# hhguo/MSMC-TTS

Hardware: AMD Instinct MI355X
Metric: mel-frames/sec MSMC-VQ-GAN train step (GAN phase) (higher is better)
Workload: dtype bf16

## Files before the change

### include/msmc_hip_debug.h

```cpp
#ifndef MSMC_HIP_DEBUG_H
#define MSMC_HIP_DEBUG_H
#include "msmc_hip.h"
#ifdef __cplusplus
extern "C" {
#endif

void msmc_vq_set_shortlist_ablate(int mask);

void msmc_vq_set_variant(int v);

void msmc_vq_wide_set_split(int wc);

void msmc_triple_wide_set_frames(int ft);

void msmc_conv_set_gather4_grid(int n);
void msmc_conv_set_gather4_grouping(int on);
void msmc_conv_set_pipeline(int on);
void msmc_conv_set_wgrad_split(int n);
void msmc_conv_set_wgrad_tpw(int n);
void msmc_conv_set_wgrad_generation(int n);
void msmc_conv_set_gather_generation(int n);
void msmc_conv_set_narrow(int on);

void msmc_conv_set_grouping(int on);

void msmc_conv_set_wgrad4_ablate(int mask);

const char* msmc_vq_last_kernel(void);
const char* msmc_loss_last_kernel(void);
void msmc_prof_enable(int on);
int msmc_prof_count(void);
int msmc_prof_read(int i, char* name, int cap, float* ms);
const char* msmc_conv_last_kernel(void);
long msmc_conv_launch_count(void);
#ifdef __cplusplus
}
#endif
#endif
```

### msmc-tts_amd/csrc/conv.hip

```cpp
#include <msmc_rt.hpp>
#include <msmc_hip.h>
#include <msmc_hip_debug.h>
#include "conv_common.inc"

extern "C" void msmc_conv_set_pipeline(int on) { msmc_conv_pipeline_enabled = on; }
static int msmc_conv_narrow_when_small = 1;
extern "C" void msmc_conv_set_narrow(int on) { msmc_conv_narrow_when_small = on; }
extern "C" const char* msmc_conv_last_kernel(void) { return msmc_conv_last; }
extern "C" long msmc_conv_launch_count(void) { return msmc_conv_launches; }
extern "C" int msmc_conv_gather(const msmc_conv_desc* d, msmc_stream stream);
static int msmc_gather_generation = 2;
extern "C" void msmc_conv_set_gather_generation(int n) { msmc_gather_generation = n; }

template <int N>
MSMC_DEV void cv_ep(float (&v)[N], const unsigned int* mk, const unsigned int* r1, const unsigned int* r2, bool has_mask,
                    bool has_res, bool has_res2, float mslope, float odiv, float oslope) {
    if (has_mask) {
#pragma unroll
        for (int j = 0; j < N; ++j) {
            const float mj = __uint_as_float((j & 1) ? (mk[j >> 1] & 0xffff0000u) : (mk[j >> 1] << 16));
            v[j] = v[j] * (mj > 0.f ? 1.f : mslope);
        }
    }
    if (has_res) {
// ... 579 lines not shown
    const bool ovec = (d.Cout % VEC) == 0;
    const size_t img = (size_t)b * d.Hout * d.Wout;
    for (int e = tid; e < 128 * BNV; e += 256) {
        const int m = e / BNV, vcol = (e - m * BNV) * VEC;
        const int po = out_off[m], co = co0 + vcol;
        if (po < 0 || co >= d.Cout) continue;
        const size_t o = (img + po) * d.Cout + co;
        float v[VEC];
#pragma unroll
        for (int q = 0; q < VEC; ++q) v[q] = ot[m * OS + vcol + q] + ((d.bias && co + q < d.Cout) ? d.bias[co + q] : 0.f);
        alignas(16) T mk[VEC], r1[VEC], r2[VEC], ov[VEC];
        if (ovec) {
            if (mask) *(u32x4*)mk = *(const u32x4*)(mask + o);
            if (res) *(u32x4*)r1 = *(const u32x4*)(res + o);
            if (res2) *(u32x4*)r2 = *(const u32x4*)(res2 + o);
        } else {
#pragma unroll
            for (int q = 0; q < VEC; ++q) {
                const bool in = co + q < d.Cout;
                if (mask) mk[q] = in ? mask[o + q] : (T)0;
                if (res) r1[q] = in ? res[o + q] : (T)0;
                if (res2) r2[q] = in ? res2[o + q] : (T)0;
            }
        }
#pragma unroll
        for (int q = 0; q < VEC; ++q) {
            float x = v[q];
            if (mask) x = x * (Elt<T>::ld(&mk[q]) > 0.f ? 1.f : d.mask_slope);
            if (res) x = x + Elt<T>::ld(&r1[q]);
            if (res2) x = Elt<T>::ld(&r2[q]) + x;
            if (d.out_div != 1.f) x = x / d.out_div;
            if (d.out_slope != 1.f) x = x > 0.f ? x : x * d.out_slope;
            Elt<T>::st(&ov[q], x);
        }
        if (ovec) {
            *(u32x4*)(out + o) = *(const u32x4*)ov;
        } else {
#pragma unroll
            for (int q = 0; q < VEC; ++q)
                if (co + q < d.Cout) out[o + q] = ov[q];
        }
    }
}


template <typename T, int NT, int CKM, int SB>
__global__ __launch_bounds__(256, 2) void conv_gather2_kernel(msmc_conv_desc d, CvGeom G) {
    cv2_body<T, NT, CKM, SB>(d, G, blockIdx.x, blockIdx.y);
}

struct CvGroupArgs {
    int n;
    int first[MSMC_GROUP_MAX + 1];
    int nx[MSMC_GROUP_MAX];
    msmc_conv_desc d[MSMC_GROUP_MAX];
    CvGeom G[MSMC_GROUP_MAX];
};
template <typename T, int NT, int CKM, int SB>
__global__ __launch_bounds__(256, 2) void conv_gather2_group_kernel(CvGroupArgs a) {
    const int k = cv_group_member(a.first, a.n);
    const int id = blockIdx.x - a.first[k];
    cv2_body<T, NT, CKM, SB>(a.d[k], a.G[k], id % a.nx[k], id / a.nx[k]);
}

template <class F>
static int cv_family_dispatch(const msmc_conv_desc* descs, const typename F::Plan* pl, const int* members, int m,
                              msmc_stream stream) {
    typename F::Args a;
    int* first = F::head(a, m);
    int blocks = 0;
    size_t lds = 0;
    for (int k = 0; k < m; ++k) {
        const int j = members[k];
        first[k] = blocks;
        F::fill(a, k, descs[j], pl[j]);
        blocks += F::blocks(pl[j]);
        if (pl[j].lds > lds) lds = pl[j].lds;
    }
    first[m] = blocks;
    ++msmc_conv_launches;
    return F::dispatch(pl[members[0]], blocks, lds, stream, m == 1 ? &descs[members[0]] : nullptr, m == 1 ? nullptr : &a);
}
template <class F>
static int cv_family_group_launch(const msmc_conv_desc* descs, int n, msmc_stream stream, bool* done) {
    typename F::Plan pl[MSMC_GROUP_LIMIT];
    bool todo[MSMC_GROUP_LIMIT];
    int count = 0;
    for (int i = 0; i < n; ++i) {
        todo[i] = !done[i] && F::mine(&descs[i]);
        count += todo[i];
    }
    if (count < F::min_members) return 0;
    for (int i = 0; i < n; ++i) {
        if (!todo[i]) continue;
        int rc = F::plan(&descs[i], &pl[i], count < MSMC_GROUP_MAX ? count : MSMC_GROUP_MAX);
        if (rc) return rc;
        if (!pl[i].applies) return MSMC_E_SHAPE;
    }
    for (int i = 0; i < n; ++i) {
        if (!todo[i]) continue;
        int members[MSMC_GROUP_MAX], m = 0;
        for (int j = i; j < n && m < MSMC_GROUP_MAX; ++j) {
            if (!todo[j] || !F::same(pl[i], pl[j])) continue;
            members[m++] = j;
            todo[j] = false;
        }
        if (m == 1 && !F::lone_single) continue;
        for (int k = 0; k < m; ++k) done[members[k]] = true;
        int rc = cv_family_dispatch<F>(descs, pl, members, m, stream);
        if (rc) return rc;
    }
    return 0;
}

#include "gather3.inc"
#include "gather4.inc"
#include "gemm1.inc"
#include "gather5.inc"
#include "gather7.inc"
#include "gather6.inc"

template <typename T, int NT, int MT>
static int cv_try_pipe(const msmc_conv_desc* d, msmc_stream stream, bool* done) {
    constexpr int XS = Elt<T>::CK + Elt<T>::VEC, CKV = Elt<T>::CK / Elt<T>::VEC;
    CvGeom G;
    size_t lds;
    *done = false;
    int rc = cv_geometry(d, &G, sizeof(T), XS, 32 * NT, &lds, CV_BM * MT);
    if (rc) return rc;
    if (lds > 160 * 1024) return 0;
    if (G.IH * G.IW * CKV > 256 * CV_XLD || d->ntaps * 32 * NT * CKV > 256 * CV_WLD) return 0;
    dim3 grid((unsigned)(G.tilesX * G.tilesY * d->B), (unsigned)((d->Cout + 32 * NT - 1) / (32 * NT)));
    rc = msmc_allow_lds((const void*)conv_gather_pipe_kernel<T, NT, MT>, (int)lds);
    if (rc) return rc;
    MSMC_LAUNCH((conv_gather_pipe_kernel<T, NT, MT>), grid, dim3(256), lds, (msmc_stream_t)stream, *d, G);
    msmc_conv_last = msmc_prof_name(msmc_kname("conv_gather_pipe_kernel", EltName<T>::v, NT, MT));
    *done = true;
    return msmc_check_launch();
}

struct Cv2Plan {
    int applies;
    int nt, ckm, sb;
    CvGeom G;
    size_t lds;
    unsigned gx, gy;
};
template <typename T>
static int cv2_plan(const msmc_conv_desc* d, Cv2Plan* pl, int* narrow_nt) {
    constexpr int XS = Elt<T>::CK + Elt<T>::VEC;
    pl->applies = 0;
    int NT = d->Cout > 32 ? 2 : 1;
    if (NT == 2 && msmc_conv_narrow_when_small) {
        const long mt = ((long)d->QH * d->QW + CV_BM - 1) / CV_BM * d->B;
        const long wide = mt * ((d->Cout + 63) / 64);
        if (wide < MSMC_NUM_CU || (wide < 2 * MSMC_NUM_CU && d->Cin >= 256)) NT = 1;
    }
    *narrow_nt = NT;
    const int gen = d->variant > 0 ? d->variant : msmc_gather_generation;
    const bool sb8 = gen == 4 || gen == 5 || (d->variant == 0 && (long)d->ntaps * 32 * NT * (Elt<T>::CK / Elt<T>::VEC) > 1024);
    const bool ck1 = gen == 3 || gen == 5 || gen == 7;
    const bool want16 = gen == 6 || gen == 7;
    bool shallow = d->Cin < 4 * Elt<T>::CK || (d->Cin % Elt<T>::VEC) != 0 || gen >= 3 || d->variant == 2;
    if (want16 && (d->Cin % Elt<T>::VEC) != 0) return MSMC_E_SHAPE;
    if (!shallow && gen == 2) {
        const long points = (long)d->B * d->QH * d->QW;
        const long ntile = (d->Cout + 32 * NT - 1) / (32 * NT);
        shallow = (points / (CV_BM * 2)) * ntile < 2 * MSMC_NUM_CU;
    }
    if (!(gen >= 2 && shallow && (long)d->Hin * d->Win * d->Cin < (1L << 31) && (long)d->Hout * d->Wout < (1L << 31)))
        return 0;
    size_t unused;
    int rc = cv_geometry(d, &pl->G, sizeof(T), XS, 32, &unused);
    if (rc) return rc;
    const long npix = (long)pl->G.IH * pl->G.IW;
    const size_t tables = (((size_t)(npix + 128 + 16) * sizeof(int)) + 15) & ~(size_t)15;
    auto lds_of = [&](int nt, int ckm) {
        const size_t xs = (size_t)Elt<T>::CK * ckm + Elt<T>::VEC;
        const size_t stage = ((size_t)npix + (size_t)d->ntaps * 32 * nt) * xs * sizeof(T);
        const size_t epi = (size_t)128 * (32 * nt + 4) * sizeof(float);
        return tables + (stage > epi ? stage : epi);
    };
    int nt = NT;
    int ckm = (d->Cin >= 2 * Elt<T>::CK && (d->Cin % Elt<T>::VEC) == 0 && lds_of(nt, 2) <= 64 * 1024 && !ck1) ? 2 : 1;
    if (lds_of(nt, ckm) > 160 * 1024 && nt == 2) nt = 1;
    const size_t lds2 = lds_of(nt, ckm);
    const long chunk_vectors = (npix + (long)d->ntaps * 32 * nt) * (Elt<T>::CK * ckm / Elt<T>::VEC);
    const bool sb16 = want16 && chunk_vectors <= 16L * 256 && (d->Cin % Elt<T>::VEC) == 0;
    if (want16 && !sb16) return MSMC_E_SHAPE;
    if (lds2 > 160 * 1024) return 0;
    pl->applies = 1;
// ... 967 lines not shown
```

### msmc-tts_amd/csrc/gather6.inc

```
#define CV6_HEAD 768
#ifndef CV6_BATCH
#define CV6_BATCH 3
#endif
struct Cv6Run {
    int npoints, ntiles;
    int nsteps;
    int pitch;
    int nco;
    int cin, cinsh;
    unsigned int m_qpi, m_qw;
    int dymin, dymax, dxmin, dxmax;
};

MSMC_DEV int cv6_div(int n, int dv, unsigned int m) {
    if (dv == 1) return n;
    unsigned int q = __umulhi((unsigned int)n, m);
    if (q * (unsigned int)dv > (unsigned int)n) --q;
    return (int)q;
}

template <int NCO>
MSMC_DEV void cv6_body(const msmc_conv_desc& d, const Cv6Run& R, const int block, const int nblocks) {
    MSMC_DYN_LDS(smem);
    typedef unsigned short T;
    const int CIN = R.cin, cinsh = R.cinsh;
    const int g8sh = cinsh >= 3 ? cinsh - 3 : 0;
    int* tapdy = (int*)smem;
    int* tapdx = tapdy + 32;
    int* koff = tapdx + 32;
    char* wimg = smem + CV6_HEAD;
    const int tid = threadIdx.x, w = wave_uniform(tid >> 6), lane = tid & 63, li = lane & 31, g = lane >> 5;
    const int Cout = d.Cout, ntaps = d.ntaps, pitch = R.pitch;
    const int nk8 = (ntaps * CIN + 7) >> 3;

    for (int e = tid; e < 32 * NCO * (pitch >> 4); e += 256) *(u32x4*)(wimg + (size_t)e * 16) = u32x4{0u, 0u, 0u, 0u};
    if (tid < 32) {
        tapdy[tid] = tid < ntaps ? d.tap_dy[tid] : 0;
        tapdx[tid] = tid < ntaps ? d.tap_dx[tid] : 0;
    }
    if (tid < 128) {
        const int t = tid >> g8sh, cg = tid - (t << g8sh);
        koff[tid] = (CIN >= 8 && t < ntaps) ? (((d.tap_dy[t] * d.Win + d.tap_dx[t]) << cinsh) + cg * 8) : 0;
    }
    __syncthreads();
    if (CIN >= 8) {
        for (int e = tid; e < Cout * nk8; e += 256) {
            const int co = e / nk8, kk = e - co * nk8;
            const int t = kk >> g8sh, cg = kk - (t << g8sh);
            const u32x4 v = *(const u32x4*)((const T*)d.w + (((size_t)d.tap_w[t] * Cout + co) << cinsh) + cg * 8);
            *(u32x4*)(wimg + (size_t)co * pitch + kk * 16) = v;
        }
    } else {
        const int kreal = ntaps << cinsh;
        for (int e = tid; e < Cout * kreal; e += 256) {
            const int co = e / kreal, k = e - co * kreal;
            const int t = k >> cinsh, ci = k - (t << cinsh);
            *(T*)(wimg + (size_t)co * pitch + k * 2) = ((const T*)d.w)[(((size_t)d.tap_w[t] * Cout + co) << cinsh) + ci];
        }
    }
    __syncthreads();

    const T* xg = (const T*)d.x;
    const float slope = d.in_slope;
    const int qpi = d.QH * d.QW;
    const T* mask = (const T*)d.mask_src;
    const T* res = (const T*)d.res;
    const T* res2 = (const T*)d.res2;
    T* out = (T*)d.out;
    const float mslope = d.mask_slope, odiv = d.out_div, oslope = d.out_slope;
    const char* wrow = wimg + (size_t)li * pitch + g * 16;

    for (int tile = block * 4 + w; tile < R.ntiles; tile += nblocks * 4) {
        const int p = tile * 32 + li;
        const bool live = p < R.npoints;
        const int pc = live ? p : R.npoints - 1;
        const int b = cv6_div(pc, qpi, R.m_qpi), q = pc - b * qpi;
        const int qy = cv6_div(q, d.QW, R.m_qw), qx = q - qy * d.QW;
        const int iy0 = d.iy0 + qy * d.isy, ix0 = d.ix0 + qx * d.isx;
        const int xb = b * d.Hin;
        const bool inside_pt = live && iy0 + R.dymin >= 0 && iy0 + R.dymax < d.Hin && ix0 + R.dxmin >= 0 && ix0 + R.dxmax < d.Win;
        const bool fast = CIN >= 8 && !wave_any(!inside_pt);
        const T* xbase = xg + (long)((xb + iy0) * d.Win + ix0) * CIN;
        f32x16 acc[NCO];
#pragma unroll
        for (int c = 0; c < NCO; ++c)
#pragma unroll
            for (int r = 0; r < 16; ++r) acc[c][r] = 0.f;
        auto load_piece = [&](int ks) -> u32x4 {
            const int kk = 2 * ks + g;
            u32x4 v = {0u, 0u, 0u, 0u};
            if (kk >= nk8) return v;
            auto pixel = [&](int t, unsigned int& off) -> bool {
                int iy = iy0 + tapdy[t], ix = ix0 + tapdx[t];
                bool inside = live;
                if (d.pad_mode == 1) {
                    iy = reflect_index(iy, d.Hin);
                    ix = reflect_index(ix, d.Win);
                } else {
                    inside = inside && (iy >= 0) && (iy < d.Hin) && (ix >= 0) && (ix < d.Win);
                }
                off = (unsigned int)(((xb + iy) * d.Win + ix) << cinsh);
                return inside;
            };
            unsigned int off;
            if (CIN >= 8) {
                const int t = kk >> g8sh, cg = kk - (t << g8sh);
                if (pixel(t, off)) v = *(const u32x4*)(xg + (size_t)off + cg * 8);
            } else if (CIN == 4) {
#pragma unroll
                for (int tp = 0; tp < 2; ++tp) {
                    const int t = 2 * kk + tp;
                    if (t < ntaps && pixel(t, off)) {
                        const u32x2 h = *(const u32x2*)(xg + (size_t)off);
                        v[2 * tp] = h[0];
                        v[2 * tp + 1] = h[1];
                    }
                }
            } else {
#pragma unroll
                for (int tp = 0; tp < 4; ++tp) {
                    const int t = 4 * kk + tp;
                    if (t < ntaps && pixel(t, off)) v[tp] = *(const unsigned int*)(xg + (size_t)off);
                }
            }
            return v;
        };
        for (int s0 = 0; s0 < R.nsteps; s0 += CV6_BATCH) {
            u32x4 xf[CV6_BATCH];
            if (fast) {
#pragma unroll
                for (int u = 0; u < CV6_BATCH; ++u) {
                    const int kk = 2 * (s0 + u) + g;
                    xf[u] = u32x4{0u, 0u, 0u, 0u};
                    if (kk < nk8) xf[u] = *(const u32x4*)(xbase + koff[kk]);
                }
            } else {
#pragma unroll
                for (int u = 0; u < CV6_BATCH; ++u) xf[u] = load_piece(s0 + u);
            }
#pragma unroll
            for (int u = 0; u < CV6_BATCH; ++u) {
                if (slope != 1.f) {
#pragma unroll
                    for (int q4 = 0; q4 < 4; ++q4) xf[u][q4] = bf16x2_leaky(xf[u][q4], slope);
                }
#pragma unroll
                for (int c = 0; c < NCO; ++c) {
                    const u32x4 wf = *(const u32x4*)(wrow + (size_t)c * 32 * pitch + (s0 + u) * 32);
                    acc[c] = mfma_bf16_32x32x16(__builtin_bit_cast(bf16x8, wf), __builtin_bit_cast(bf16x8, xf[u]), acc[c]);
                }
            }
        }
#pragma unroll
        for (int c = 0; c < NCO; ++c) cv5_swap_runs(acc[c]);
        if (!live) continue;
        const size_t opix = ((size_t)b * d.Hout + d.oy0 + qy * d.osy) * d.Wout + d.ox0 + qx * d.osx;
#pragma unroll
        for (int c = 0; c < NCO; ++c) {
#pragma unroll
            for (int h = 0; h < 2; ++h) {
                const int n = 32 * c + 16 * h + 8 * g;
                if (n >= Cout) continue;
                const size_t o = opix * Cout + n;
                if (n + 4 == Cout && !(Cout & 3)) {
                    f32x4 b0 = {0.f, 0.f, 0.f, 0.f};
                    if (d.bias) b0 = *(const f32x4*)(d.bias + n);
                    u32x2 mk = {0u, 0u}, r1 = mk, r2 = mk;
                    if (mask) mk = *(const u32x2*)(mask + o);
                    if (res) r1 = *(const u32x2*)(res + o);
                    if (res2) r2 = *(const u32x2*)(res2 + o);
                    float ov[4];
#pragma unroll
                    for (int j = 0; j < 4; ++j) ov[j] = acc[c][8 * h + j] + b0[j];
                    {
                        const unsigned int mkw[2] = {mk[0], mk[1]}, r1w[2] = {r1[0], r1[1]}, r2w[2] = {r2[0], r2[1]};
                        cv_ep<4>(ov, mkw, r1w, r2w, mask != nullptr, res != nullptr, res2 != nullptr, mslope, odiv, oslope);
                    }
                    const u32x2 pk = {pack_bf16x2(ov[0], ov[1]), pack_bf16x2(ov[2], ov[3])};
                    *(u32x2*)(out + o) = pk;
                    continue;
                }
                if (n + 8 > Cout || (Cout & 7)) {
                    for (int j = 0; j < 8 && n + j < Cout; ++j) {
                        float v = acc[c][8 * h + j] + (d.bias ? d.bias[n + j] : 0.f);
                        if (mask) v = v * (bf16_bits_to_f32(mask[o + j]) > 0.f ? 1.f : mslope);
                        if (res) v = v + bf16_bits_to_f32(res[o + j]);
                        if (res2) v = bf16_bits_to_f32(res2[o + j]) + v;
                        if (odiv != 1.f) v = v / odiv;
                        if (oslope != 1.f) v = v > 0.f ? v : v * oslope;
                        out[o + j] = f32_to_bf16_bits(v);
                    }
                    continue;
                }
                f32x4 b0 = {0.f, 0.f, 0.f, 0.f}, b1 = b0;
                if (d.bias) {
                    b0 = *(const f32x4*)(d.bias + n);
                    b1 = *(const f32x4*)(d.bias + n + 4);
                }
                u32x4 mk = {0u, 0u, 0u, 0u}, r1 = mk, r2 = mk;
                if (mask) mk = *(const u32x4*)(mask + o);
                if (res) r1 = *(const u32x4*)(res + o);
                if (res2) r2 = *(const u32x4*)(res2 + o);
                float ov[8];
#pragma unroll
                for (int j = 0; j < 8; ++j) ov[j] = acc[c][8 * h + j] + (j < 4 ? b0[j & 3] : b1[j & 3]);
                {
                    const unsigned int mkw[4] = {mk[0], mk[1], mk[2], mk[3]}, r1w[4] = {r1[0], r1[1], r1[2], r1[3]},
                                       r2w[4] = {r2[0], r2[1], r2[2], r2[3]};
                    cv_ep<8>(ov, mkw, r1w, r2w, mask != nullptr, res != nullptr, res2 != nullptr, mslope, odiv, oslope);
                }
                const u32x4 pk = {pack_bf16x2(ov[0], ov[1]), pack_bf16x2(ov[2], ov[3]), pack_bf16x2(ov[4], ov[5]), pack_bf16x2(ov[6], ov[7])};
                *(u32x4*)(out + o) = pk;
            }
        }
    }
}

template <int NCO>
__global__ __launch_bounds__(256) void conv_gather6_kernel(msmc_conv_desc d, Cv6Run R) {
    cv6_body<NCO>(d, R, (int)blockIdx.x, (int)gridDim.x);
}
struct Cv6GroupArgs {
    int n;
    int first[MSMC_GROUP_MAX + 1];
    msmc_conv_desc d[MSMC_GROUP_MAX];
    Cv6Run R[MSMC_GROUP_MAX];
};
template <int NCO>
__global__ __launch_bounds__(256) void conv_gather6_group_kernel(Cv6GroupArgs a) {
    const int k = cv_group_member(a.first, a.n);
    cv6_body<NCO>(a.d[k], a.R[k], (int)blockIdx.x - a.first[k], a.first[k + 1] - a.first[k]);
}

struct Cv6Plan {
    int applies;
    Cv6Run R;
    size_t lds;
    int blocks;
};
static bool cv6_is_variant(int variant) { return variant == 50; }

static int cv6_plan(const msmc_conv_desc* d, Cv6Plan* pl, int share = 1) {
    pl->applies = 0;
    if (d->dtype != 1 || !cv6_is_variant(d->variant)) return 0;
    if (d->Cin != 2 && d->Cin != 4 && d->Cin != 8 && d->Cin != 16 && d->Cin != 32 && d->Cin != 64) return 0;
    if (d->Cout <= 0 || d->Cout > 64 || d->ntaps <= 0 || d->ntaps > 32 || d->Cin * d->ntaps > 704) return 0;
    if (d->Cin < 8 && ((size_t)d->x & (size_t)(d->Cin * 2 - 1))) return 0;
    if (!(d->in_slope >= 0.f && d->in_slope <= 1.f)) return 0;
    if (((size_t)d->x | (size_t)d->w | (size_t)d->out | (size_t)d->res | (size_t)d->res2 | (size_t)d->mask_src | (size_t)d->bias) & 15)
        return 0;
    const long npoints = (long)d->B * d->QH * d->QW;
    if (npoints <= 0 || npoints >= (1L << 31)) return 0;
    if ((long)d->B * d->Hin * d->Win * d->Cin >= (1L << 31) || (long)d->B * d->Hout * d->Wout * d->Cout >= (1L << 31)) return 0;
    Cv6Run& R = pl->R;
    R.npoints = (int)npoints;
    R.ntiles = (int)((npoints + 31) / 32);
    const int k = d->Cin * d->ntaps;
    R.nsteps = (((k + 15) / 16 + CV6_BATCH - 1) / CV6_BATCH) * CV6_BATCH;
    R.pitch = ((R.nsteps * 32 + 255) & ~255) + 16;
    R.nco = d->Cout > 32 ? 2 : 1;
    R.cin = d->Cin;
    R.cinsh = d->Cin == 2 ? 1 : d->Cin == 4 ? 2 : d->Cin == 8 ? 3 : d->Cin == 16 ? 4 : d->Cin == 32 ? 5 : 6;
    R.m_qpi = (unsigned int)((1ULL << 32) / (unsigned long long)((long)d->QH * d->QW)) + 1u;
    R.m_qw = (unsigned int)((1ULL << 32) / (unsigned long long)d->QW) + 1u;
    pl->lds = CV6_HEAD + (size_t)32 * R.nco * R.pitch;
    R.dymin = R.dymax = d->tap_dy[0];
    R.dxmin = R.dxmax = d->tap_dx[0];
    for (int t = 1; t < d->ntaps; ++t) {
        if (d->tap_dy[t] < R.dymin) R.dymin = d->tap_dy[t];
        if (d->tap_dy[t] > R.dymax) R.dymax = d->tap_dy[t];
        if (d->tap_dx[t] < R.dxmin) R.dxmin = d->tap_dx[t];
        if (d->tap_dx[t] > R.dxmax) R.dxmax = d->tap_dx[t];
    }
    if (pl->lds > 96 * 1024) return 0;
    long nb = (long)(4 * MSMC_NUM_CU) / (share > 0 ? share : 1);
    const long maxb = (R.ntiles + 3) / 4;
    if (nb > maxb) nb = maxb;
    if (nb < 1) nb = 1;
    pl->blocks = (int)nb;
    pl->applies = 1;
    return 0;
}

static int cv6_dispatch(const Cv6Plan& pl, int blocks, size_t lds, msmc_stream stream, const msmc_conv_desc* d,
                        const Cv6GroupArgs* group) {
    int rc;
#define CV6_GO(KERNEL_, NC_, ...)                                                                                  \
    do {                                                                                                           \
        rc = msmc_allow_lds((const void*)KERNEL_<NC_>, (int)lds);                                                  \
        if (rc) return rc;                                                                                         \
        MSMC_LAUNCH((KERNEL_<NC_>), dim3((unsigned)blocks), dim3(256), lds, (msmc_stream_t)stream, __VA_ARGS__);   \
    } while (0)
    if (!group && pl.R.nco == 1) CV6_GO(conv_gather6_kernel, 1, *d, pl.R);
    else if (!group) CV6_GO(conv_gather6_kernel, 2, *d, pl.R);
    else if (pl.R.nco == 1) CV6_GO(conv_gather6_group_kernel, 1, *group);
    else CV6_GO(conv_gather6_group_kernel, 2, *group);
#undef CV6_GO
    static thread_local char name[64];
    snprintf(name, sizeof(name), "%s<%d>", group ? "conv_gather6_group_kernel" : "conv_gather6_kernel", pl.R.nco);
    msmc_conv_last = msmc_prof_name(name);
    return msmc_check_launch();
}

static int cv6_launch(const msmc_conv_desc* d, msmc_stream stream) {
    Cv6Plan pl;
    int rc = cv6_plan(d, &pl);
    if (rc) return rc;
    if (!pl.applies) return 0;
    return cv_launched(cv6_dispatch(pl, pl.blocks, pl.lds, stream, d, nullptr));
}

struct Cv6Family {
    typedef Cv6Plan Plan;
    typedef Cv6GroupArgs Args;
    static constexpr int min_members = 1;
    static constexpr bool lone_single = true;
    static bool mine(const msmc_conv_desc* d) { return cv6_is_variant(d->variant); }
    static int plan(const msmc_conv_desc* d, Plan* pl, int share) { return cv6_plan(d, pl, share); }
    static bool same(const Plan& p, const Plan& q) { return p.R.nco == q.R.nco; }
    static int blocks(const Plan& p) { return p.blocks; }
    static int* head(Args& a, int m) { a.n = m; return a.first; }
    static void fill(Args& a, int k, const msmc_conv_desc& d, const Plan& p) {
        a.d[k] = d;
        a.R[k] = p.R;
    }
    static int dispatch(const Plan& p, int blocks, size_t lds, msmc_stream stream, const msmc_conv_desc* d, const Args* group) {
        return cv6_dispatch(p, blocks, lds, stream, d, group);
    }
};
```

### msmc-tts_amd/msmctts_amd/hip/lib.py

```python
import ctypes
import os

import torch

_HERE = os.path.dirname(os.path.abspath(__file__))
DEFAULT_PATH = os.path.normpath(os.path.join(_HERE, '..', '..', 'lib', 'libmsmc_hip.so'))
DEFAULT_PATH = os.environ.get('MSMC_HIP_LIB', DEFAULT_PATH)

_lib = None
_host_pointers_ok = False

_vp, _i, _f, _sz = ctypes.c_void_p, ctypes.c_int, ctypes.c_float, ctypes.c_size_t

_SIGNATURES = {
    'msmc_backend': (ctypes.c_char_p, []),
    'msmc_abi_version': (_i, []),
    'msmc_stream_create': (_i, [ctypes.POINTER(ctypes.c_void_p)]),
    'msmc_stream_destroy': (_i, [_vp]),
    'msmc_vq_prepare': (_i, [_vp, _vp, _vp, _i, _i, _i, _vp]),
    'msmc_vq_search': (_i, [_vp, _vp, _vp, _vp, _vp, _vp, _i, _i, _i, _i, _vp]),
    'msmc_vq_search_stream': (_i, [_vp, _vp, _vp, _vp, _vp, _vp, _i, _i, _i, _i, _i, _vp]),
    'msmc_vq_search_wide': (_i, [_vp, _vp, _vp, _vp, _vp, _vp, _i, _i, _i, _vp]),
    'msmc_vq_assign_wide': (_i, [_vp, _vp, _vp, _vp, _vp, _i, _i, _i, _vp]),
    'msmc_vq_shortlist_bytes': (_sz, [_i, _i, _i]),
# ... 114 lines not shown
    'msmc_attn_fwd_f32': (_i, [_vp, _vp, _vp, _vp, _i, _i, _i, _i, _f, _f, _vp, ctypes.c_longlong, _vp]),
    'msmc_attn_bwd_f32': (_i, [_vp, _vp, _vp, _vp, _vp, _vp, _vp, _i, _i, _i, _i, _f, _f, _vp, ctypes.c_longlong, _vp]),
    'msmc_wn_prepare_multi': (_i, [_vp, _i, _i, _vp]),
    'msmc_wn_prepare_multi_tiled': (_i, [_vp, _i, _i, _i, _vp]),
    'msmc_wn_tile_blocks': (_i, [_i, _i, _i]),
    'msmc_wn_prepare_multi_tiles': (_i, [_vp, _i, _i, _i, _i, _vp, _vp, _i, _vp, _vp]),
    'msmc_wn_backward_multi': (_i, [_vp, _i, _i, _vp]),
    'msmc_wn_backward_multi_acc': (_i, [_vp, _i, _i, _i, _vp]),
    'msmc_wn_backward_multi_rows': (_i, [_vp, _i, _i, _i, _i, _vp]),
    'msmc_reflect_fold_multi': (_i, [ctypes.POINTER(_vp), ctypes.POINTER(_vp), ctypes.POINTER(_vp), ctypes.POINTER(_i), ctypes.POINTER(_i), ctypes.POINTER(_i),
                                ctypes.POINTER(_i), _i, _i, _f, _i, _vp]),
    'msmc_reflect_fold_multi_res': (_i, [ctypes.POINTER(_vp), ctypes.POINTER(_vp), ctypes.POINTER(_vp), ctypes.POINTER(_vp), ctypes.POINTER(_i),
                                    ctypes.POINTER(_i), ctypes.POINTER(_i), ctypes.POINTER(_i), _i, _i, _f, _i, _vp]),
    'msmc_reflect_fold_multi_tap': (_i, [ctypes.POINTER(_vp), ctypes.POINTER(_vp), ctypes.POINTER(_vp), ctypes.POINTER(_vp), ctypes.POINTER(_i),
                                    ctypes.POINTER(_i), ctypes.POINTER(_i), ctypes.POINTER(_i), _i, _i, _f, _i, _vp]),
    'msmc_lrelu_bwd_multi': (_i, [ctypes.POINTER(_vp), ctypes.POINTER(_vp), ctypes.POINTER(_vp), ctypes.POINTER(ctypes.c_long), _i, _f, _i, _vp]),
    'msmc_colsum': (_i, [_vp, _vp, ctypes.c_long, _i, _i, _vp]),
    'msmc_colsum_workspace': (_sz, [ctypes.c_long, _i]),
    'msmc_colsum_ws': (_i, [_vp, _vp, ctypes.c_long, _i, _i, _i, _vp, _sz, _vp]),
    'msmc_add_ln_fwd': (_i, [_vp, _vp, _vp, _vp, _vp, _vp, _vp, _vp, _vp, ctypes.c_long, _i, _f, _f, _vp, ctypes.c_longlong,
                        _i, _vp]),
    'msmc_fc_add_ln_fwd': (_i, [_vp, _vp, _vp, _vp, _vp, _vp, _vp, _vp, _vp, _vp, _vp, ctypes.c_long, _i, _i, _f, _f, _vp,
                           ctypes.c_longlong, _vp]),
    'msmc_add_ln_bwd_workspace': (_sz, [ctypes.c_long, _i]),
    'msmc_add_ln_param_multi': (_i, [_vp, _i, _vp]),
    'msmc_add_ln_bwd': (_i, [_vp, _vp, _vp, _vp, _vp, _vp, _vp, _vp, _vp, _vp, _vp, _sz, ctypes.c_long, _i, _f, _vp,
                        ctypes.c_longlong, _i, _i, _vp]),
    'msmc_fft_prologue': (_i, [_vp, _vp, _i, _vp, _i, _vp, _vp, _vp, _i, _i, _i, _i, _i, _i, _vp]),
    'msmc_gate_fwd': (_i, [_vp, _vp, ctypes.c_long, _i, _f, _vp, ctypes.c_longlong, _i, _vp]),
    'msmc_gate_bwd': (_i, [_vp, _vp, _vp, ctypes.c_long, _i, _f, _vp, ctypes.c_longlong, _i, _vp]),
    'msmc_sum_n': (_i, [_vp, _vp, _vp, _vp, _vp, ctypes.c_long, _i, _vp]),
    'msmc_dropout_add_fwd': (_i, [_vp, _vp, _vp, ctypes.c_long, _f, _vp, ctypes.c_longlong, _i, _vp]),
    'msmc_dropout_bwd': (_i, [_vp, _vp, ctypes.c_long, _f, _vp, ctypes.c_longlong, _i, _vp]),
    'msmc_row_mask': (_i, [_vp, _i, _vp, _i, _i, _i, _vp]),
    'msmc_tanh_fwd': (_i, [_vp, _vp, ctypes.c_long, _i, _vp]),
    'msmc_tanh_bwd': (_i, [_vp, _vp, _vp, ctypes.c_long, _i, _vp]),
    'msmc_tanh_f32_fwd': (_i, [_vp, _vp, ctypes.c_long, _i, _vp]),
    'msmc_tanh_f32_bwd': (_i, [_vp, _vp, _vp, ctypes.c_long, _i, _vp]),
    'msmc_bn_workspace': (_sz, [ctypes.c_long, _i]),
    'msmc_bn_fwd': (_i, [_vp, _vp, _vp, _vp, _vp, _vp, _vp, _vp, _sz, ctypes.c_long, _i, _f, _f, _i, _i, _vp]),
    'msmc_bn_eval_fwd': (_i, [_vp, _vp, _vp, _vp, _vp, ctypes.c_long, _i, _f, _i, _i, _vp]),
    'msmc_bn_bwd': (_i, [_vp, _vp, _vp, _vp, _vp, _vp, _sz, ctypes.c_long, _i, _i, _i, _vp]),
    'msmc_bn_eval_bwd': (_i, [_vp, _vp, _vp, ctypes.c_long, _i, _i, _i, _vp]),
    'msmc_relu_bn_workspace': (_sz, [ctypes.c_long, _i]),
    'msmc_relu_bn_fwd': (_i, [_vp, ctypes.c_long, _vp, _vp, _vp, ctypes.c_long, _vp, _vp, _vp, _vp, _vp, _vp, _sz, ctypes.c_long, _i,
                         _f, _f, _i, _vp]),
    'msmc_relu_bn_eval_fwd': (_i, [_vp, ctypes.c_long, _vp, _vp, _vp, _vp, _vp, ctypes.c_long, _vp, ctypes.c_long, _i, _f, _i, _vp]),
    'msmc_relu_bn_bwd': (_i, [_vp, ctypes.c_long, _vp, ctypes.c_long, _vp, _vp, _vp, _vp, ctypes.c_long, _vp, _vp, _vp, _sz,
                         ctypes.c_long, _i, _i, _vp]),
    'msmc_relu_bn_eval_bwd': (_i, [_vp, ctypes.c_long, _vp, ctypes.c_long, _vp, _vp, _vp, _vp, ctypes.c_long, _vp, _vp, _vp, _sz,
                              ctypes.c_long, _i, _i, _vp]),
    'msmc_se_workspace': (_sz, [_i, _i, _i]),
    'msmc_se_fwd': (_i, [_vp, _vp, _vp, _vp, _vp, _vp, _vp, _vp, _vp, _vp, _vp, _sz, _i, _i, _i, _i, _vp]),
    'msmc_se_bwd_gate': (_i, [_vp, _vp, _vp, _vp, _sz, _i, _i, _i, _i, _vp]),
    'msmc_se_bwd_apply': (_i, [_vp, _vp, _vp, _vp, _i, _i, _i, _i, _vp]),
    'msmc_asp_workspace': (_sz, [_i, _i, _i]),
    'msmc_asp_fwd': (_i, [_vp, _vp, _vp, _vp, _vp, _sz, _i, _i, _i, _i, _vp]),
    'msmc_asp_bwd': (_i, [_vp, _vp, _vp, _vp, _vp, _vp, _i, _i, _i, _i, _vp]),
    'msmc_opt_chunk': (_i, []),
    'msmc_opt_clip_adamw': (_i, [_vp, _i, _i, _f, _vp, _vp, _vp, _vp, _f, _f, _f, _f, _i, _vp]),
    'msmc_lrelu_bwd': (_i, [_vp, _vp, _vp, ctypes.c_long, _f, _i, _vp]),
    'msmc_reflect_fold': (_i, [_vp, _vp, _vp, _i, _i, _i, _i, _i, _f, _i, _vp]),
})

_DEBUG_SIGNATURES = {
    'msmc_vq_last_kernel': (ctypes.c_char_p, []),
    'msmc_loss_last_kernel': (ctypes.c_char_p, []),
    'msmc_conv_last_kernel': (ctypes.c_char_p, []),
    'msmc_conv_launch_count': (ctypes.c_long, []),
    'msmc_prof_enable': (None, [_i]),
    'msmc_prof_count': (_i, []),
    'msmc_prof_read': (_i, [_i, ctypes.c_char_p, _i, ctypes.POINTER(ctypes.c_float)]),
    'msmc_vq_set_shortlist_ablate': (None, [_i]),
    'msmc_vq_set_variant': (None, [_i]),
    'msmc_vq_wide_set_split': (None, [_i]),
    'msmc_triple_wide_set_frames': (None, [_i]),
    'msmc_conv_set_grouping': (None, [_i]),
    'msmc_conv_set_pipeline': (None, [_i]),
    'msmc_conv_set_wgrad_split': (None, [_i]),
    'msmc_conv_set_wgrad_generation': (None, [_i]),
    'msmc_conv_set_wgrad4_ablate': (None, [_i]),
    'msmc_conv_set_gather4_grid': (None, [_i]),
    'msmc_conv_set_gather4_grouping': (None, [_i]),
    'msmc_conv_set_gather_generation': (None, [_i]),
    'msmc_conv_set_narrow': (None, [_i]),
    'msmc_conv_set_wgrad_tpw': (None, [_i]),
}


class LnParamItem(ctypes.Structure):
    _fields_ = [('part', ctypes.c_void_p), ('dgamma', ctypes.c_void_p), ('dbeta', ctypes.c_void_p), ('nblocks', ctypes.c_int),
                ('C', ctypes.c_int), ('accumulate', ctypes.c_int), ('reserved', ctypes.c_int)]


def exported_symbols():
    return sorted(_SIGNATURES)


def debug_symbols():
    return sorted(_DEBUG_SIGNATURES)


def _bind(handle):
    for name, (res, args) in list(_SIGNATURES.items()) + list(_DEBUG_SIGNATURES.items()):
        fn = getattr(handle, name)
        fn.restype = res
        fn.argtypes = args
    return handle


def load(path=None):
    path = DEFAULT_PATH if path is None else path
    if not os.path.isfile(path):
        raise RuntimeError(
            'msmctts_amd: HIP extension %s not found. Build it with `python -c "import __graft_entry__ as g; '
            'g.build()"` (hipcc --offload-arch=gfx950). There is no CPU fallback.' % path)
    return _bind(ctypes.CDLL(path))


def get():
    global _lib
    if _lib is None:
        _lib = load()
    return _lib


def use_library_for_tests(path):
    global _lib, _host_pointers_ok
    _lib = load(path)
    _host_pointers_ok = _lib.msmc_backend() == b'emu'
    return _lib


def backend():
    return get().msmc_backend().decode()


def ptr(t, dtype=None):
    if t is None:
        return None
    if dtype is not None and t.dtype != dtype:
        raise TypeError('expected %s, got %s' % (dtype, t.dtype))
    if not t.is_contiguous():
        raise ValueError('msmc HIP ops take contiguous tensors')
    if not t.is_cuda and not _host_pointers_ok:
        raise RuntimeError('msmc HIP ops run on the GPU only (got a %s tensor); there is no CPU path' % t.device)
    return ctypes.c_void_p(t.data_ptr())


def stream(t):
    if t.is_cuda:
        return ctypes.c_void_p(torch.cuda.current_stream(t.device).cuda_stream)
    return ctypes.c_void_p(0)


def check(rc, what):
    if rc != 0:
        raise RuntimeError('%s failed with code %d' % (what, rc))


def call(name, *args, what=None):
    check(getattr(get(), name)(*args), what or name)


def workspace(nbytes, device, have=None, floor=0):
    if have is not None and have.numel() * have.element_size() >= nbytes:
# ... 3 lines not shown
```

Measured before the change: 336,900.

## Software-pipeline gather6 conv tiles, stage bias in LDS, rebalance grouped blocks

```diff
diff --git a/include/msmc_hip_debug.h b/include/msmc_hip_debug.h
--- a/include/msmc_hip_debug.h
+++ b/include/msmc_hip_debug.h
@@ -15,6 +15,8 @@
 
 void msmc_conv_set_gather4_grid(int n);
 void msmc_conv_set_gather4_grouping(int on);
+void msmc_conv_set_gather6_blocks(int n);
+void msmc_conv_set_gather6_even_split(int on);
 void msmc_conv_set_pipeline(int on);
 void msmc_conv_set_wgrad_split(int n);
 void msmc_conv_set_wgrad_tpw(int n);
@@ -33,6 +35,7 @@
 int msmc_prof_read(int i, char* name, int cap, float* ms);
 const char* msmc_conv_last_kernel(void);
 long msmc_conv_launch_count(void);
+int msmc_conv_gather6_last_grid(int* blocks, int cap);
 #ifdef __cplusplus
 }
 #endif
diff --git a/msmc-tts_amd/csrc/conv.hip b/msmc-tts_amd/csrc/conv.hip
--- a/msmc-tts_amd/csrc/conv.hip
+++ b/msmc-tts_amd/csrc/conv.hip
@@ -685,6 +685,12 @@
     return F::dispatch(pl[members[0]], blocks, lds, stream, m == 1 ? &descs[members[0]] : nullptr, m == 1 ? nullptr : &a);
 }
 template <class F>
+static auto cv_family_rebalance(typename F::Plan* pl, const int* members, int m, int) -> decltype(F::rebalance(pl, members, m)) {
+    F::rebalance(pl, members, m);
+}
+template <class F>
+static void cv_family_rebalance(typename F::Plan*, const int*, int, long) {}
+template <class F>
 static int cv_family_group_launch(const msmc_conv_desc* descs, int n, msmc_stream stream, bool* done) {
     typename F::Plan pl[MSMC_GROUP_LIMIT];
     bool todo[MSMC_GROUP_LIMIT];
@@ -710,6 +716,7 @@
         }
         if (m == 1 && !F::lone_single) continue;
         for (int k = 0; k < m; ++k) done[members[k]] = true;
+        cv_family_rebalance<F>(pl, members, m, 0);
         int rc = cv_family_dispatch<F>(descs, pl, members, m, stream);
         if (rc) return rc;
     }
diff --git a/msmc-tts_amd/csrc/gather6.inc b/msmc-tts_amd/csrc/gather6.inc
--- a/msmc-tts_amd/csrc/gather6.inc
+++ b/msmc-tts_amd/csrc/gather6.inc
@@ -1,4 +1,5 @@
 #define CV6_HEAD 768
+#define CV6_BIAS 256
 #ifndef CV6_BATCH
 #define CV6_BATCH 3
 #endif
@@ -29,6 +30,7 @@
     int* tapdx = tapdy + 32;
     int* koff = tapdx + 32;
     char* wimg = smem + CV6_HEAD;
+    float* biasl = (float*)(wimg + (size_t)32 * NCO * R.pitch);
     const int tid = threadIdx.x, w = wave_uniform(tid >> 6), lane = tid & 63, li = lane & 31, g = lane >> 5;
     const int Cout = d.Cout, ntaps = d.ntaps, pitch = R.pitch;
     const int nk8 = (ntaps * CIN + 7) >> 3;
@@ -38,6 +40,7 @@
         tapdy[tid] = tid < ntaps ? d.tap_dy[tid] : 0;
         tapdx[tid] = tid < ntaps ? d.tap_dx[tid] : 0;
     }
+    if (tid < CV6_BIAS / 4) biasl[tid] = (d.bias && tid < d.Cout) ? d.bias[tid] : 0.f;
     if (tid < 128) {
         const int t = tid >> g8sh, cg = tid - (t << g8sh);
         koff[tid] = (CIN >= 8 && t < ntaps) ? (((d.tap_dy[t] * d.Win + d.tap_dx[t]) << cinsh) + cg * 8) : 0;
@@ -70,154 +73,220 @@
     const float mslope = d.mask_slope, odiv = d.out_div, oslope = d.out_slope;
     const char* wrow = wimg + (size_t)li * pitch + g * 16;
 
-    for (int tile = block * 4 + w; tile < R.ntiles; tile += nblocks * 4) {
+    struct Tile {
+        int iy0, ix0, xb;
+        bool live, fast;
+        const T* xbase;
+        size_t opix;
+    };
+    struct Ep {
+        u32x4 mk, r1, r2;
+    };
+    constexpr bool EP_AHEAD = NCO == 1;
+    auto tile_setup = [&](int tile) -> Tile {
+        Tile t;
         const int p = tile * 32 + li;
-        const bool live = p < R.npoints;
-        const int pc = live ? p : R.npoints - 1;
+        t.live = p < R.npoints;
+        const int pc = t.live ? p : R.npoints - 1;
         const int b = cv6_div(pc, qpi, R.m_qpi), q = pc - b * qpi;
         const int qy = cv6_div(q, d.QW, R.m_qw), qx = q - qy * d.QW;
-        const int iy0 = d.iy0 + qy * d.isy, ix0 = d.ix0 + qx * d.isx;
-        const int xb = b * d.Hin;
-        const bool inside_pt = live && iy0 + R.dymin >= 0 && iy0 + R.dymax < d.Hin && ix0 + R.dxmin >= 0 && ix0 + R.dxmax < d.Win;
-        const bool fast = CIN >= 8 && !wave_any(!inside_pt);
-        const T* xbase = xg + (long)((xb + iy0) * d.Win + ix0) * CIN;
-        f32x16 acc[NCO];
-#pragma unroll
-        for (int c = 0; c < NCO; ++c)
-#pragma unroll
-            for (int r = 0; r < 16; ++r) acc[c][r] = 0.f;
-        auto load_piece = [&](int ks) -> u32x4 {
-            const int kk = 2 * ks + g;
-            u32x4 v = {0u, 0u, 0u, 0u};
-            if (kk >= nk8) return v;
-            auto pixel = [&](int t, unsigned int& off) -> bool {
-                int iy = iy0 + tapdy[t], ix = ix0 + tapdx[t];
-                bool inside = live;
-                if (d.pad_mode == 1) {
-                    iy = reflect_index(iy, d.Hin);
-                    ix = reflect_index(ix, d.Win);
-                } else {
-                    inside = inside && (iy >= 0) && (iy < d.Hin) && (ix >= 0) && (ix < d.Win);
+        t.iy0 = d.iy0 + qy * d.isy;
+        t.ix0 = d.ix0 + qx * d.isx;
+        t.xb = b * d.Hin;
+        const bool inside_pt = t.live && t.iy0 + R.dymin >= 0 && t.iy0 + R.dymax < d.Hin && t.ix0 + R.dxmin >= 0 && t.ix0 + R.dxmax < d.Win;
+        t.fast = CIN >= 8 && !wave_any(!inside_pt);
+        t.xbase = xg + (long)((t.xb + t.iy0) * d.Win + t.ix0) * CIN;
+        t.opix = ((size_t)b * d.Hout + d.oy0 + qy * d.osy) * d.Wout + d.ox0 + qx * d.osx;
+        return t;
+    };
+    auto load_piece = [&](const Tile& t, int ks) -> u32x4 {
+        const int kk = 2 * ks + g;
+        u32x4 v = {0u, 0u, 0u, 0u};
+        if (kk >= nk8) return v;
+        auto pixel = [&](int tp, unsigned int& off) -> bool {
+            int iy = t.iy0 + tapdy[tp], ix = t.ix0 + tapdx[tp];
+            bool inside = t.live;
+            if (d.pad_mode == 1) {
+                iy = reflect_index(iy, d.Hin);
+                ix = reflect_index(ix, d.Win);
+            } else {
+                inside = inside && (iy >= 0) && (iy < d.Hin) && (ix >= 0) && (ix < d.Win);
+            }
+            off = (unsigned int)(((t.xb + iy) * d.Win + ix) << cinsh);
+            return inside;
+        };
+        unsigned int off;
+        if (CIN >= 8) {
+            const int tp = kk >> g8sh, cg = kk - (tp << g8sh);
+            if (pixel(tp, off)) v = *(const u32x4*)(xg + (size_t)off + cg * 8);
+        } else if (CIN == 4) {
+#pragma unroll
+            for (int u = 0; u < 2; ++u) {
+                const int tp = 2 * kk + u;
+                if (tp < ntaps && pixel(tp, off)) {
+                    const u32x2 h = *(const u32x2*)(xg + (size_t)off);
+                    v[2 * u] = h[0];
+                    v[2 * u + 1] = h[1];
                 }
-                off = (unsigned int)(((xb + iy) * d.Win + ix) << cinsh);
-                return inside;
-            };
-            unsigned int off;
-            if (CIN >= 8) {
-                const int t = kk >> g8sh, cg = kk - (t << g8sh);
-                if (pixel(t, off)) v = *(const u32x4*)(xg + (size_t)off + cg * 8);
-            } else if (CIN == 4) {
-#pragma unroll
-                for (int tp = 0; tp < 2; ++tp) {
-                    const int t = 2 * kk + tp;
-                    if (t < ntaps && pixel(t, off)) {
-                        const u32x2 h = *(const u32x2*)(xg + (size_t)off);
-                        v[2 * tp] = h[0];
-                        v[2 * tp + 1] = h[1];
-                    }
-                }
-            } else {
-#pragma unroll
-                for (int tp = 0; tp < 4; ++tp) {
-                    const int t = 4 * kk + tp;
-                    if (t < ntaps && pixel(t, off)) v[tp] = *(const unsigned int*)(xg + (size_t)off);
-                }
-            }
-            return v;
-        };
-        for (int s0 = 0; s0 < R.nsteps; s0 += CV6_BATCH) {
-            u32x4 xf[CV6_BATCH];
-            if (fast) {
-#pragma unroll
-                for (int u = 0; u < CV6_BATCH; ++u) {
-                    const int kk = 2 * (s0 + u) + g;
-                    xf[u] = u32x4{0u, 0u, 0u, 0u};
-                    if (kk < nk8) xf[u] = *(const u32x4*)(xbase + koff[kk]);
-                }
-            } else {
-#pragma unroll
-                for (int u = 0; u < CV6_BATCH; ++u) xf[u] = load_piece(s0 + u);
-            }
+            }
+        } else {
+#pragma unroll
+            for (int u = 0; u < 4; ++u) {
+                const int tp = 4 * kk + u;
+                if (tp < ntaps && pixel(tp, off)) v[u] = *(const unsigned int*)(xg + (size_t)off);
+            }
+        }
+        return v;
+    };
+    auto load_batch = [&](const Tile& t, int s0, u32x4 (&xf)[CV6_BATCH]) {
+        if (t.fast) {
 #pragma unroll
             for (int u = 0; u < CV6_BATCH; ++u) {
+                const int kk = 2 * (s0 + u) + g;
+                xf[u] = *(const u32x4*)(t.xbase + koff[kk < nk8 ? kk : nk8 - 1]);
+            }
+        } else {
+#pragma unroll
+            for (int u = 0; u < CV6_BATCH; ++u) xf[u] = load_piece(t, s0 + u);
+        }
+    };
+    auto ep_form = [&](int n) -> int {
+        if (n >= Cout) return 0;
+        if (n + 4 == Cout && !(Cout & 3)) return 1;
+        if (n + 8 > Cout || (Cout & 7)) return 2;
+        return 3;
+    };
+    auto ep_fetch = [&](const Tile& t, int c, int h) -> Ep {
+        Ep e;
+        e.mk = u32x4{0u, 0u, 0u, 0u};
+        e.r1 = e.mk;
+        e.r2 = e.mk;
+        const int n = 32 * c + 16 * h + 8 * g;
+        const int form = ep_form(n);
+        if (!t.live) return e;
+        const size_t o = t.opix * Cout + n;
+        if (form == 1) {
+            if (mask) { const u32x2 v = *(const u32x2*)(mask + o); e.mk[0] = v[0]; e.mk[1] = v[1]; }
+            if (res) { const u32x2 v = *(const u32x2*)(res + o); e.r1[0] = v[0]; e.r1[1] = v[1]; }
+            if (res2) { const u32x2 v = *(const u32x2*)(res2 + o); e.r2[0] = v[0]; e.r2[1] = v[1]; }
+        } else if (form == 3) {
+            if (mask) e.mk = *(const u32x4*)(mask + o);
+            if (res) e.r1 = *(const u32x4*)(res + o);
+            if (res2) e.r2 = *(const u32x4*)(res2 + o);
+        }
+        return e;
+    };
+
+    const int stride = nblocks * 4;
+    int tile = block * 4 + w;
+    if (tile >= R.ntiles) return;
+    Tile ld = tile_setup(tile), cur = ld;
+    int s0 = 0;
+    u32x4 xe[CV6_BATCH], xo[CV6_BATCH];
+    f32x16 acc[NCO];
+#pragma unroll
+    for (int c = 0; c < NCO; ++c)
+#pragma unroll
+        for (int r = 0; r < 16; ++r) acc[c][r] = 0.f;
+    load_batch(ld, 0, xe);
+    auto step = [&](u32x4 (&xc)[CV6_BATCH], u32x4 (&xn)[CV6_BATCH]) -> bool {
+        const bool last = s0 + CV6_BATCH >= R.nsteps;
+        const int next = tile + stride;
+        const bool more = next < R.ntiles;
+        Ep ep[1][2];
+        if (last) {
+#pragma unroll
+            for (int h = 0; h < 2; ++h)
+                if (EP_AHEAD) ep[0][h] = ep_fetch(cur, 0, h);
+            if (more) ld = tile_setup(next);
+        }
+        auto mma_batch = [&]() {
+#pragma unroll
+            for (int u = 0; u < CV6_BATCH; ++u) {
+                if (2 * (s0 + u) + g >= nk8) xc[u] = u32x4{0u, 0u, 0u, 0u};
                 if (slope != 1.f) {
 #pragma unroll
-                    for (int q4 = 0; q4 < 4; ++q4) xf[u][q4] = bf16x2_leaky(xf[u][q4], slope);
+                    for (int q4 = 0; q4 < 4; ++q4) xc[u][q4] = bf16x2_leaky(xc[u][q4], slope);
                 }
 #pragma unroll
                 for (int c = 0; c < NCO; ++c) {
                     const u32x4 wf = *(const u32x4*)(wrow + (size_t)c * 32 * pitch + (s0 + u) * 32);
-                    acc[c] = mfma_bf16_32x32x16(__builtin_bit_cast(bf16x8, wf), __builtin_bit_cast(bf16x8, xf[u]), acc[c]);
+                    acc[c] = mfma_bf16_32x32x16(__builtin_bit_cast(bf16x8, wf), __builtin_bit_cast(bf16x8, xc[u]), acc[c]);
                 }
             }
+        };
+        if (!last || more) load_batch(ld, last ? 0 : s0 + CV6_BATCH, xn);
+        mma_batch();
+        if (!last) {
+            s0 += CV6_BATCH;
+            return true;
         }
 #pragma unroll
         for (int c = 0; c < NCO; ++c) cv5_swap_runs(acc[c]);
-        if (!live) continue;
-        const size_t opix = ((size_t)b * d.Hout + d.oy0 + qy * d.osy) * d.Wout + d.ox0 + qx * d.osx;
-#pragma unroll
-        for (int c = 0; c < NCO; ++c) {
-#pragma unroll
-            for (int h = 0; h < 2; ++h) {
-                const int n = 32 * c + 16 * h + 8 * g;
-                if (n >= Cout) continue;
-                const size_t o = opix * Cout + n;
-                if (n + 4 == Cout && !(Cout & 3)) {
-                    f32x4 b0 = {0.f, 0.f, 0.f, 0.f};
-                    if (d.bias) b0 = *(const f32x4*)(d.bias + n);
-                    u32x2 mk = {0u, 0u}, r1 = mk, r2 = mk;
-                    if (mask) mk = *(const u32x2*)(mask + o);
-                    if (res) r1 = *(const u32x2*)(res + o);
-                    if (res2) r2 = *(const u32x2*)(res2 + o);
-                    float ov[4];
-#pragma unroll
-                    for (int j = 0; j < 4; ++j) ov[j] = acc[c][8 * h + j] + b0[j];
+        if (cur.live) {
+#pragma unroll
+            for (int c = 0; c < NCO; ++c) {
+#pragma unroll
+                for (int h = 0; h < 2; ++h) {
+                    const int n = 32 * c + 16 * h + 8 * g;
+                    const int form = ep_form(n);
+                    if (form == 0) continue;
+                    const size_t o = cur.opix * Cout + n;
+                    const Ep e = EP_AHEAD ? ep[0][h] : ep_fetch(cur, c, h);
+                    if (form == 1) {
+                        const f32x4 b0 = *(const f32x4*)(biasl + n);
+                        float ov[4];
+#pragma unroll
+                        for (int j = 0; j < 4; ++j) ov[j] = acc[c][8 * h + j] + b0[j];
+                        {
+                            const unsigned int mkw[2] = {e.mk[0], e.mk[1]}, r1w[2] = {e.r1[0], e.r1[1]}, r2w[2] = {e.r2[0], e.r2[1]};
+                            cv_ep<4>(ov, mkw, r1w, r2w, mask != nullptr, res != nullptr, res2 != nullptr, mslope, odiv, oslope);
+                        }
+                        const u32x2 pk = {pack_bf16x2(ov[0], ov[1]), pack_bf16x2(ov[2], ov[3])};
+                        *(u32x2*)(out + o) = pk;
+                        continue;
+                    }
+                    if (form == 2) {
+                        for (int j = 0; j < 8 && n + j < Cout; ++j) {
+                            float v = acc[c][8 * h + j] + biasl[n + j];
+                            if (mask) v = v * (bf16_bits_to_f32(mask[o + j]) > 0.f ? 1.f : mslope);
+                            if (res) v = v + bf16_bits_to_f32(res[o + j]);
+                            if (res2) v = bf16_bits_to_f32(res2[o + j]) + v;
+                            if (odiv != 1.f) v = v / odiv;
+                            if (oslope != 1.f) v = v > 0.f ? v : v * oslope;
+                            out[o + j] = f32_to_bf16_bits(v);
+                        }
+                        continue;
+                    }
+                    const f32x4 b0 = *(const f32x4*)(biasl + n), b1 = *(const f32x4*)(biasl + n + 4);
+                    float ov[8];
+#pragma unroll
+                    for (int j = 0; j < 8; ++j) ov[j] = acc[c][8 * h + j] + (j < 4 ? b0[j & 3] : b1[j & 3]);
                     {
-                        const unsigned int mkw[2] = {mk[0], mk[1]}, r1w[2] = {r1[0], r1[1]}, r2w[2] = {r2[0], r2[1]};
-                        cv_ep<4>(ov, mkw, r1w, r2w, mask != nullptr, res != nullptr, res2 != nullptr, mslope, odiv, oslope);
+                        const unsigned int mkw[4] = {e.mk[0], e.mk[1], e.mk[2], e.mk[3]}, r1w[4] = {e.r1[0], e.r1[1], e.r1[2], e.r1[3]},
+                                           r2w[4] = {e.r2[0], e.r2[1], e.r2[2], e.r2[3]};
+                        cv_ep<8>(ov, mkw, r1w, r2w, mask != nullptr, res != nullptr, res2 != nullptr, mslope, odiv, oslope);
                     }
-                    const u32x2 pk = {pack_bf16x2(ov[0], ov[1]), pack_bf16x2(ov[2], ov[3])};
-                    *(u32x2*)(out + o) = pk;
-                    continue;
+                    const u32x4 pk = {pack_bf16x2(ov[0], ov[1]), pack_bf16x2(ov[2], ov[3]), pack_bf16x2(ov[4], ov[5]), pack_bf16x2(ov[6], ov[7])};
+                    *(u32x4*)(out + o) = pk;
                 }
-                if (n + 8 > Cout || (Cout & 7)) {
-                    for (int j = 0; j < 8 && n + j < Cout; ++j) {
-                        float v = acc[c][8 * h + j] + (d.bias ? d.bias[n + j] : 0.f);
-                        if (mask) v = v * (bf16_bits_to_f32(mask[o + j]) > 0.f ? 1.f : mslope);
-                        if (res) v = v + bf16_bits_to_f32(res[o + j]);
-                        if (res2) v = bf16_bits_to_f32(res2[o + j]) + v;
-                        if (odiv != 1.f) v = v / odiv;
-                        if (oslope != 1.f) v = v > 0.f ? v : v * oslope;
-                        out[o + j] = f32_to_bf16_bits(v);
-                    }
-                    continue;
-                }
-                f32x4 b0 = {0.f, 0.f, 0.f, 0.f}, b1 = b0;
-                if (d.bias) {
-                    b0 = *(const f32x4*)(d.bias + n);
-                    b1 = *(const f32x4*)(d.bias + n + 4);
-                }
-                u32x4 mk = {0u, 0u, 0u, 0u}, r1 = mk, r2 = mk;
-                if (mask) mk = *(const u32x4*)(mask + o);
-                if (res) r1 = *(const u32x4*)(res + o);
-                if (res2) r2 = *(const u32x4*)(res2 + o);
-                float ov[8];
-#pragma unroll
-                for (int j = 0; j < 8; ++j) ov[j] = acc[c][8 * h + j] + (j < 4 ? b0[j & 3] : b1[j & 3]);
-                {
-                    const unsigned int mkw[4] = {mk[0], mk[1], mk[2], mk[3]}, r1w[4] = {r1[0], r1[1], r1[2], r1[3]},
-                                       r2w[4] = {r2[0], r2[1], r2[2], r2[3]};
-                    cv_ep<8>(ov, mkw, r1w, r2w, mask != nullptr, res != nullptr, res2 != nullptr, mslope, odiv, oslope);
-                }
-                const u32x4 pk = {pack_bf16x2(ov[0], ov[1]), pack_bf16x2(ov[2], ov[3]), pack_bf16x2(ov[4], ov[5]), pack_bf16x2(ov[6], ov[7])};
-                *(u32x4*)(out + o) = pk;
-            }
-        }
-    }
+            }
+        }
+        if (!more) return false;
+        cur = ld;
+        tile = next;
+        s0 = 0;
+#pragma unroll
+        for (int c = 0; c < NCO; ++c)
+#pragma unroll
+            for (int r = 0; r < 16; ++r) acc[c][r] = 0.f;
+        return true;
+    };
+    while (step(xe, xo) && step(xo, xe)) {}
 }
 
 template <int NCO>
-__global__ __launch_bounds__(256) void conv_gather6_kernel(msmc_conv_desc d, Cv6Run R) {
+__global__ __launch_bounds__(256, 4) void conv_gather6_kernel(msmc_conv_desc d, Cv6Run R) {
     cv6_body<NCO>(d, R, (int)blockIdx.x, (int)gridDim.x);
 }
 struct Cv6GroupArgs {
@@ -227,7 +296,7 @@
     Cv6Run R[MSMC_GROUP_MAX];
 };
 template <int NCO>
-__global__ __launch_bounds__(256) void conv_gather6_group_kernel(Cv6GroupArgs a) {
+__global__ __launch_bounds__(256, 4) void conv_gather6_group_kernel(Cv6GroupArgs a) {
     const int k = cv_group_member(a.first, a.n);
     cv6_body<NCO>(a.d[k], a.R[k], (int)blockIdx.x - a.first[k], a.first[k + 1] - a.first[k]);
 }
@@ -239,6 +308,19 @@
     int blocks;
 };
 static bool cv6_is_variant(int variant) { return variant == 50; }
+static int msmc_cv6_block_cap = 0;
+extern "C" void msmc_conv_set_gather6_blocks(int n) { msmc_cv6_block_cap = n; }
+static long cv6_max_blocks(const Cv6Run& R) {
+    long maxb = (R.ntiles + 3) / 4;
+    if (msmc_cv6_block_cap > 0 && maxb > msmc_cv6_block_cap) maxb = msmc_cv6_block_cap;
+    return maxb;
+}
+static thread_local int msmc_cv6_last_n = 0;
+static thread_local int msmc_cv6_last_blocks[MSMC_GROUP_MAX];
+extern "C" int msmc_conv_gather6_last_grid(int* blocks, int cap) {
+    for (int k = 0; k < msmc_cv6_last_n && k < cap; ++k) blocks[k] = msmc_cv6_last_blocks[k];
+    return msmc_cv6_last_n;
+}
 
 static int cv6_plan(const msmc_conv_desc* d, Cv6Plan* pl, int share = 1) {
     pl->applies = 0;
@@ -273,13 +355,66 @@
         if (d->tap_dx[t] > R.dxmax) R.dxmax = d->tap_dx[t];
     }
     if (pl->lds > 96 * 1024) return 0;
+    pl->lds += CV6_BIAS;
     long nb = (long)(4 * MSMC_NUM_CU) / (share > 0 ? share : 1);
-    const long maxb = (R.ntiles + 3) / 4;
+    const long maxb = cv6_max_blocks(R);
     if (nb > maxb) nb = maxb;
     if (nb < 1) nb = 1;
     pl->blocks = (int)nb;
     pl->applies = 1;
     return 0;
+}
+
+static int msmc_cv6_even_split = 0;
+extern "C" void msmc_conv_set_gather6_even_split(int on) { msmc_cv6_even_split = on; }
+static void cv6_rebalance(Cv6Plan* pl, const int* members, int m) {
+    if (m < 2 || msmc_cv6_even_split) return;
+    long work[MSMC_GROUP_MAX], cap[MSMC_GROUP_MAX], nb[MSMC_GROUP_MAX];
+    bool fixed[MSMC_GROUP_MAX];
+    long budget = 0;
+    for (int k = 0; k < m; ++k) {
+        const Cv6Run& R = pl[members[k]].R;
+        work[k] = (long)R.ntiles * R.nsteps * R.nco;
+        cap[k] = cv6_max_blocks(R);
+        budget += pl[members[k]].blocks;
+        fixed[k] = false;
+        nb[k] = 0;
+    }
+    for (int round = 0; round < m; ++round) {
+        long left = budget, total = 0;
+        for (int k = 0; k < m; ++k) {
+            if (fixed[k]) left -= nb[k];
+            else total += work[k];
+        }
+        if (total <= 0) break;
+        if (left < 0) left = 0;
+        bool clamped = false;
+        for (int k = 0; k < m; ++k) {
+            if (fixed[k]) continue;
+            nb[k] = left * work[k] / total;
+            if (nb[k] >= cap[k]) {
+                nb[k] = cap[k];
+                fixed[k] = clamped = true;
+            } else if (nb[k] < 1) {
+                nb[k] = 1;
+                fixed[k] = clamped = true;
+            }
+        }
+        if (!clamped) break;
+    }
+    long sum = 0;
+    for (int k = 0; k < m; ++k) sum += nb[k];
+    while (sum != budget) {
+        int best = -1;
+        for (int k = 0; k < m; ++k) {
+            if (sum < budget ? nb[k] >= cap[k] : nb[k] <= 1) continue;
+            if (best < 0 || (sum < budget ? work[k] * nb[best] > work[best] * nb[k] : work[k] * nb[best] < work[best] * nb[k])) best = k;
+        }
+        if (best < 0) break;
+        nb[best] += sum < budget ? 1 : -1;
+        sum += sum < budget ? 1 : -1;
+    }
+    for (int k = 0; k < m; ++k) pl[members[k]].blocks = (int)nb[k];
 }
 
 static int cv6_dispatch(const Cv6Plan& pl, int blocks, size_t lds, msmc_stream stream, const msmc_conv_desc* d,
@@ -296,6 +431,8 @@
     else if (pl.R.nco == 1) CV6_GO(conv_gather6_group_kernel, 1, *group);
     else CV6_GO(conv_gather6_group_kernel, 2, *group);
 #undef CV6_GO
+    msmc_cv6_last_n = group ? group->n : 1;
+    for (int k = 0; k < msmc_cv6_last_n; ++k) msmc_cv6_last_blocks[k] = group ? group->first[k + 1] - group->first[k] : blocks;
     static thread_local char name[64];
     snprintf(name, sizeof(name), "%s<%d>", group ? "conv_gather6_group_kernel" : "conv_gather6_kernel", pl.R.nco);
     msmc_conv_last = msmc_prof_name(name);
@@ -319,6 +456,7 @@
     static int plan(const msmc_conv_desc* d, Plan* pl, int share) { return cv6_plan(d, pl, share); }
     static bool same(const Plan& p, const Plan& q) { return p.R.nco == q.R.nco; }
     static int blocks(const Plan& p) { return p.blocks; }
+    static void rebalance(Plan* pl, const int* members, int m) { cv6_rebalance(pl, members, m); }
     static int* head(Args& a, int m) { a.n = m; return a.first; }
     static void fill(Args& a, int k, const msmc_conv_desc& d, const Plan& p) {
         a.d[k] = d;
diff --git a/msmc-tts_amd/msmctts_amd/hip/lib.py b/msmc-tts_amd/msmctts_amd/hip/lib.py
--- a/msmc-tts_amd/msmctts_amd/hip/lib.py
+++ b/msmc-tts_amd/msmctts_amd/hip/lib.py
@@ -220,6 +220,9 @@
     'msmc_conv_set_wgrad4_ablate': (None, [_i]),
     'msmc_conv_set_gather4_grid': (None, [_i]),
     'msmc_conv_set_gather4_grouping': (None, [_i]),
+    'msmc_conv_set_gather6_blocks': (None, [_i]),
+    'msmc_conv_set_gather6_even_split': (None, [_i]),
+    'msmc_conv_gather6_last_grid': (_i, [ctypes.POINTER(_i), _i]),
     'msmc_conv_set_gather_generation': (None, [_i]),
     'msmc_conv_set_narrow': (None, [_i]),
     'msmc_conv_set_wgrad_tpw': (None, [_i]),
```

Result: no change. 334,600 (-0.7%).
